# jaak-s/libfastsparse

Measured on AMD Instinct MI355X. Metric: fp64 CSR SpMV effective GB/s (% HBM3E peak), higher is better.
Workload: dtype f64

## Files before the change

### libfastsparse_amd/csrc/fs_kernels_twopass.hip

```cpp
#include <stdlib.h>

#include "fs_kernel_util.h"

namespace fs {


template <bool VALUED, int U, bool NTLD, bool NTST, int BC>
__device__ __forceinline__ void expand_share(double *__restrict__ xband, int ncol, int B, const unsigned *__restrict__ band_ptr,
                                             const uint16_t *__restrict__ lcol, const double *__restrict__ vals,
                                             const unsigned *__restrict__ gdst, const double *__restrict__ x, int xs,
                                             double *__restrict__ prod, unsigned g0, unsigned g1)
{
  const int t = threadIdx.x;
  if (g0 >= g1) return;
  int b;
  {
    int lo = 0, hi = B - 1;
    while (lo < hi) {
      const int mid = lo + ((hi - lo + 1) >> 1);
      if (band_ptr[mid] <= g0) lo = mid; else hi = mid - 1;
    }
    b = lo;
  }
  for (unsigned g = g0; g < g1; ++b) {
    const unsigned gb = band_ptr[b + 1] < g1 ? band_ptr[b + 1] : g1;
    if (gb <= g) continue;
    const int c0 = b * BC;
    const int w = (ncol - c0 < BC) ? ncol - c0 : BC;
    __syncthreads();
    {
      double r[BC / kBinBlock];
#pragma unroll
      for (int j = 0; j < BC / kBinBlock; ++j) {
        const int i = j * kBinBlock + t;
        r[j] = __builtin_nontemporal_load(x + (int64_t)(c0 + (i < w ? i : w - 1)) * xs);
      }
#pragma unroll
      for (int j = 0; j < BC / kBinBlock; ++j) {
        const int i = j * kBinBlock + t;
        xband[i] = (i < w) ? r[j] : 0.0;
      }
      if (t < 8) xband[BC + t] = 0.0;
    }
    __syncthreads();
    const int64_t e0 = (int64_t)g * kBinGroup, e1 = (int64_t)gb * kBinGroup;
    constexpr int64_t kRound = 2 * U * kBinBlock;
    int64_t o = e0 + 2 * t;
    for (; o - 2 * t + kRound <= e1; o += kRound) {
      unsigned a[U], d[U];
      v2d v[U];
#pragma unroll
      for (int k = 0; k < U; ++k) {
        const int64_t e = o + (int64_t)k * 2 * kBinBlock;
        a[k] = stream_load<NTLD>((const unsigned *)(lcol + e));
        d[k] = stream_load<NTLD>(gdst + (e >> kBinGroupLog));
        if (VALUED) v[k] = stream_load<NTLD>((const v2d *)(vals + e));
      }
      __builtin_amdgcn_sched_barrier(0);
#pragma unroll
      for (int k = 0; k < U; ++k) {
        const int64_t e = o + (int64_t)k * 2 * kBinBlock;
        v2d p = {xband[a[k] & 0xffffu], xband[a[k] >> 16]};
        if (VALUED) { p.x *= v[k].x; p.y *= v[k].y; }
        stream_store<NTST>(p, (v2d *)(prod + (int64_t)d[k] * kBinGroup + (e & (kBinGroup - 1))));
      }
    }
    for (; o < e1; o += 2 * kBinBlock) {
      const unsigned a = stream_load<NTLD>((const unsigned *)(lcol + o));
      const unsigned d = stream_load<NTLD>(gdst + (o >> kBinGroupLog));
      v2d p = {xband[a & 0xffffu], xband[a >> 16]};
      if (VALUED) {
        const v2d v = stream_load<NTLD>((const v2d *)(vals + o));
        p.x *= v.x; p.y *= v.y;
      }
      stream_store<NTST>(p, (v2d *)(prod + (int64_t)d * kBinGroup + (o & (kBinGroup - 1))));
    }
    g = gb;
  }
}

template <bool VALUED, int U, bool NTLD, bool NTST, int BC = kBinCols>
__global__ __launch_bounds__(kBinBlock) void spmv_expand_kernel(
    int ncol, int B, const unsigned *__restrict__ band_ptr, const uint16_t *__restrict__ lcol,
    const double *__restrict__ vals, const unsigned *__restrict__ gdst, const double *__restrict__ x, int xs,
    double *__restrict__ prod, unsigned gbeg, unsigned gend)
{
  __shared__ double xband[BC + 8];
  const uint64_t groups = gend - gbeg;
  const unsigned g0 = gbeg + (unsigned)(groups * blockIdx.x / gridDim.x), g1 = gbeg + (unsigned)(groups * (blockIdx.x + 1) / gridDim.x);
  expand_share<VALUED, U, NTLD, NTST, BC>(xband, ncol, B, band_ptr, lcol, vals, gdst, x, xs, prod, g0, g1);
}

template <bool NTLD, bool L8>
__device__ __forceinline__ v4u row_ids_load(const uint16_t *__restrict__ lrow, const uint8_t *__restrict__ lrow8,
                                            const uint16_t *__restrict__ gbase, int64_t e)
{
  if (!L8) return stream_load<NTLD>((const v4u *)(lrow + e));
  typedef unsigned v2u __attribute__((ext_vector_type(2)));
  const v2u d = stream_load<NTLD>((const v2u *)(lrow8 + e));
  return v4u{d.x, d.y, (unsigned)gbase[e >> kBinGroupLog], (unsigned)(e >> 3) & 1u};
}

template <bool L8>
__device__ __forceinline__ v4u row_ids(v4u raw)
{
  if (!L8) return raw;
  const unsigned dx = raw.x, dy = raw.y;
  const unsigned s0 = dx & 0xffu, s1 = s0 + ((dx >> 8) & 0xffu), s2 = s1 + ((dx >> 16) & 0xffu), s3 = s2 + (dx >> 24);
  const unsigned s4 = s3 + (dy & 0xffu), s5 = s4 + ((dy >> 8) & 0xffu), s6 = s5 + ((dy >> 16) & 0xffu), s7 = s6 + (dy >> 24);
  const unsigned below = (unsigned)__builtin_amdgcn_update_dpp(0, (int)s7, 0x111 , 0xf, 0xf, false);
  const unsigned off = raw.z + (raw.w ? below : 0u);
  return v4u{(off + s0) | ((off + s1) << 16), (off + s2) | ((off + s3) << 16), (off + s4) | ((off + s5) << 16), (off + s6) | ((off + s7) << 16)};
}

template <bool L8>
__device__ __forceinline__ unsigned line_ids_load(const uint16_t *__restrict__ lrow, const uint8_t *__restrict__ lrow8,
                                                  const uint16_t *__restrict__ gbase, int64_t e)
{
  if (!L8) return *(const unsigned *)(lrow + e);
  return (unsigned)*(const uint16_t *)(lrow8 + e) | ((unsigned)gbase[e >> kBinGroupLog] << 16);
}

template <bool L8>
__device__ __forceinline__ unsigned line_ids(unsigned raw)
{
  if (!L8) return raw;
  const unsigned d0 = raw & 0xffu, own = d0 + ((raw >> 8) & 0xffu), l = threadIdx.x & 7u;
  unsigned s = own, u;
  u = (unsigned)__builtin_amdgcn_update_dpp(0, (int)s, 0x111 , 0xf, 0xf, false); s += l >= 1 ? u : 0u;
  u = (unsigned)__builtin_amdgcn_update_dpp(0, (int)s, 0x112 , 0xf, 0xf, false); s += l >= 2 ? u : 0u;
  u = (unsigned)__builtin_amdgcn_update_dpp(0, (int)s, 0x114 , 0xf, 0xf, false); s += l >= 4 ? u : 0u;
  const unsigned off = (raw >> 16) + s - own;
  return (off + d0) | ((off + own) << 16);
}

template <bool NTLD, bool L8 = false>
__device__ __forceinline__ void reduce_panel(double *__restrict__ ytile, int panel, const unsigned *__restrict__ bin_ptr,
                                             const int *__restrict__ panel_row, const uint16_t *__restrict__ lrow,
                                             const double *__restrict__ prod, double *__restrict__ y, int ys,
                                             const uint8_t *__restrict__ lrow8 = nullptr, const uint16_t *__restrict__ gbase = nullptr)
{
  const int t = threadIdx.x;
  const int r0 = panel_row[panel], nr = panel_row[panel + 1] - r0;
  for (int i = t; i < nr; i += kBinBlock) ytile[i] = 0.0;
  __syncthreads();
  const int64_t e0 = (int64_t)bin_ptr[panel] * kBinGroup, e1 = (int64_t)bin_ptr[panel + 1] * kBinGroup;
#define FS_ADD(idx, val) __hip_atomic_fetch_add(&ytile[idx], val, __ATOMIC_RELAXED, __HIP_MEMORY_SCOPE_WORKGROUP)
#define FS_ADD2(A, P) FS_ADD((A) & 0xffffu, (P).x); FS_ADD((A) >> 16, (P).y);
  constexpr int64_t kStep = 8 * kBinBlock, kRound = 2 * kStep;
  const int wave0 = (t >> 6) * 512, lane0 = wave0 + 2 * (t & 63);
  int64_t eb = e0;
  for (; eb + kRound <= e1; eb += kRound) {
    const int64_t e = eb + lane0;
    unsigned a[2][4];
    v2d p[2][4];
#pragma unroll
    for (int k = 0; k < 2; ++k)
#pragma unroll
      for (int j = 0; j < 4; ++j) {
        const int64_t ek = e + k * kStep + 128 * j;
        a[k][j] = line_ids_load<L8>(lrow, lrow8, gbase, ek);
        p[k][j] = stream_load<NTLD>((const v2d *)(prod + ek));
      }
    __builtin_amdgcn_sched_barrier(0);
#pragma unroll
    for (int k = 0; k < 2; ++k)
#pragma unroll
      for (int j = 0; j < 4; ++j) {
        const unsigned r = line_ids<L8>(a[k][j]);
        FS_ADD2(r, p[k][j])
      }
  }
  for (; eb + wave0 < e1; eb += kStep) {
    const int64_t e = eb + lane0;
    unsigned a[4];
    v2d p[4];
#pragma unroll
    for (int j = 0; j < 4; ++j) {
      const int64_t ej = e + 128 * j, ec = ej < e1 ? ej : e1 - 2;
      a[j] = line_ids_load<L8>(lrow, lrow8, gbase, ec);
      p[j] = stream_load<NTLD>((const v2d *)(prod + ec));
    }
#pragma unroll
    for (int j = 0; j < 4; ++j) {
      const unsigned r = line_ids<L8>(a[j]);
      if (e + 128 * j < e1) { FS_ADD2(r, p[j]) }
    }
  }
#undef FS_ADD2
#undef FS_ADD
  __syncthreads();
  for (int i = t; i < nr; i += kBinBlock) y[(int64_t)(r0 + i) * ys] = ytile[i];
}

template <bool NTLD, int RM = kBinRowsMax, bool L8 = false>
__global__ __launch_bounds__(kBinBlock) void spmv_reduce_kernel(
    const unsigned *__restrict__ bin_ptr, const int *__restrict__ panel_row, const uint16_t *__restrict__ lrow,
    const double *__restrict__ prod, double *__restrict__ y, int ys, int pbase, const uint8_t *__restrict__ lrow8 = nullptr,
    const uint16_t *__restrict__ gbase = nullptr)
{
  __shared__ double ytile[RM];
  reduce_panel<NTLD, L8>(ytile, pbase + blockIdx.x, bin_ptr, panel_row, lrow, prod, y, ys, lrow8, gbase);
}

#ifndef FS_ORDERED_DEPTH
#define FS_ORDERED_DEPTH 16
#endif
template <bool NTLD, int RM, int DEPTH, bool L8 = false>
__global__ __launch_bounds__(64) void spmv_reduce_ordered_kernel(
    const unsigned *__restrict__ bin_ptr, const int *__restrict__ panel_row, const uint16_t *__restrict__ lrow,
    const double *__restrict__ prod, double *__restrict__ y, int ys, int pbase, const uint8_t *__restrict__ lrow8 = nullptr,
    const uint16_t *__restrict__ gbase = nullptr)
{
  __shared__ __attribute__((aligned(16))) double ytile[RM];
  const int t = threadIdx.x;
  const int panel = pbase + blockIdx.x;
  const int r0 = panel_row[panel], nr = panel_row[panel + 1] - r0;
  for (int i = 2 * t; i < nr; i += 128) *reinterpret_cast<v2d *>(&ytile[i]) = v2d{0.0, 0.0};
  const int64_t e0 = (int64_t)bin_ptr[panel] * kBinGroup, e1 = (int64_t)bin_ptr[panel + 1] * kBinGroup;
#define FS_ADD(idx, val) __hip_atomic_fetch_add(&ytile[idx], val, __ATOMIC_RELAXED, __HIP_MEMORY_SCOPE_WORKGROUP)
#define FS_ADD8(A, P)                                                  \
  FS_ADD(A.x & 0xffffu, P[0].x); FS_ADD(A.x >> 16, P[0].y);            \
  FS_ADD(A.y & 0xffffu, P[1].x); FS_ADD(A.y >> 16, P[1].y);            \
  FS_ADD(A.z & 0xffffu, P[2].x); FS_ADD(A.z >> 16, P[2].y);            \
  FS_ADD(A.w & 0xffffu, P[3].x); FS_ADD(A.w >> 16, P[3].y);
  constexpr int64_t kStep = 8 * 64;
  v4u a[DEPTH];
  v2d p[DEPTH][4];
  auto fetch = [&](int k, int64_t e) {
    const int64_t ec = (e + 8 <= e1) ? e : (e1 - e0 >= 8 ? e1 - 8 : e0);
    a[k] = row_ids_load<NTLD, L8>(lrow, lrow8, gbase, ec);
#pragma unroll
    for (int j = 0; j < 4; ++j) p[k][j] = stream_load<NTLD>((const v2d *)(prod + ec + 2 * j));
  };
  if (e1 > e0) {
    int64_t e = e0 + 8 * t;
#pragma unroll
    for (int k = 0; k < DEPTH; ++k) fetch(k, e + (int64_t)k * kStep);
    for (; e - 8 * t < e1; e += (int64_t)DEPTH * kStep) {
#pragma unroll
      for (int k = 0; k < DEPTH; ++k) {
        const int64_t ek = e + (int64_t)k * kStep;
        const v4u ak = row_ids<L8>(a[k]);
        v2d pk[4] = {p[k][0], p[k][1], p[k][2], p[k][3]};
        fetch(k, ek + (int64_t)DEPTH * kStep);
        if (ek + 8 <= e1) { FS_ADD8(ak, pk) }
      }
    }
  }
#undef FS_ADD8
#undef FS_ADD
  __syncthreads();
  for (int i = t; i < nr; i += 64) y[(int64_t)(r0 + i) * ys] = ytile[i];
}

template <bool VALUED, int BC, int NACC, bool ORDERED>
__global__ __launch_bounds__(kBinBlock) void spmv_longrows_kernel(
    int ncol, int B, int nlong, const int64_t *__restrict__ band_ptr, const unsigned *__restrict__ seg_ptr,
    const uint16_t *__restrict__ lcol, const uint16_t *__restrict__ lrow, const double *__restrict__ vals,
    const double *__restrict__ x, int xs, double *__restrict__ ylong, double *__restrict__ ypart)
{
  __shared__ double xband[BC + 8];
  __shared__ double acc[NACC];
  const int t = threadIdx.x, lane = t & 63, wave = t >> 6;
  for (int i = t; i < nlong; i += kBinBlock) acc[i] = 0.0;
  const int64_t pairs = band_ptr[B] >> 1;
  const int64_t e_beg = 2 * (pairs * blockIdx.x / gridDim.x), e_end = 2 * (pairs * (blockIdx.x + 1) / gridDim.x);
  if (e_beg < e_end) {
    int b;
    {
      int lo = 0, hi = B - 1;
      while (lo < hi) {
        const int mid = lo + ((hi - lo + 1) >> 1);
        if (band_ptr[mid] <= e_beg) lo = mid; else hi = mid - 1;
      }
      b = lo;
    }
    double rn[BC / kBinBlock];
    int have = -1;
    auto request = [&](int bb) {
      const int cb = bb * BC;
      const int wb = (ncol - cb < BC) ? ncol - cb : BC;
#pragma unroll
      for (int j = 0; j < BC / kBinBlock; ++j) {
        const int i = j * kBinBlock + t;
        rn[j] = __builtin_nontemporal_load(x + (int64_t)(cb + (i < wb ? i : wb - 1)) * xs);
      }
      have = bb;
    };
    auto wave_step = [&](int64_t o, bool live, int64_t oc) {
      const unsigned a = *reinterpret_cast<const unsigned *>(lcol + oc);
      const unsigned rr = *reinterpret_cast<const unsigned *>(lrow + oc);
      v2d p = {xband[a & 0xffffu], xband[a >> 16]};
      if (VALUED) { const v2d v = *reinterpret_cast<const v2d *>(vals + oc); p.x *= v.x; p.y *= v.y; }
      unsigned key = 0xffffffffu;
      double sum = 0.0;
      if (live) {
        const unsigned r0 = rr & 0xffffu, r1 = rr >> 16;
        if (r0 == r1) { key = r0; sum = p.x + p.y; }
        else { __hip_atomic_fetch_add(&acc[r0], p.x, __ATOMIC_RELAXED, __HIP_MEMORY_SCOPE_WORKGROUP); key = r1; sum = p.y; }
      }
#pragma unroll
      for (int d = 1; d < 64; d <<= 1) {
        const unsigned ku = __shfl_up(key, d);
        const double su = __shfl_up(sum, d);
        if (lane >= d && ku == key) sum += su;
      }
      const unsigned kn = __shfl_down(key, 1);
      if (live && (lane == 63 || kn != key))
        __hip_atomic_fetch_add(&acc[key], sum, __ATOMIC_RELAXED, __HIP_MEMORY_SCOPE_WORKGROUP);
      (void)o;
    };
    for (int64_t e = e_beg; e < e_end; ++b) {
      const int64_t eb = band_ptr[b + 1] < e_end ? band_ptr[b + 1] : e_end;
      if (eb <= e) continue;
      const int c0 = b * BC;
      const int w = (ncol - c0 < BC) ? ncol - c0 : BC;
      if (have != b) request(b);
      __syncthreads();
#pragma unroll
      for (int j = 0; j < BC / kBinBlock; ++j) {
        const int i = j * kBinBlock + t;
        xband[i] = (i < w) ? rn[j] : 0.0;
      }
      if (t < 8) xband[BC + t] = 0.0;
      __syncthreads();
      if (b + 1 < B && eb < e_end) request(b + 1);
      if (ORDERED) {
        const int64_t s0 = band_ptr[b] + seg_ptr[b * (kLongOwners + 1) + wave], s1 = band_ptr[b] + seg_ptr[b * (kLongOwners + 1) + wave + 1];
        const int64_t lo = s0 > e ? s0 : e, hi = s1 < eb ? s1 : eb;
        for (int64_t o0 = lo; o0 < hi; o0 += 128) {
          const int64_t o = o0 + 2 * lane;
          const bool live = o < hi;
          wave_step(o, live, live ? o : lo);
        }
      } else {
        for (int64_t o0 = e; o0 < eb; o0 += 2 * kBinBlock) {
          const int64_t o = o0 + 2 * t;
          const bool live = o < eb;
          wave_step(o, live, live ? o : e);
        }
      }
      e = eb;
    }
  }
  __syncthreads();
  if (ORDERED) {
    double *__restrict__ mine = ypart + (int64_t)blockIdx.x * nlong;
    for (int i = t; i < nlong; i += kBinBlock) mine[i] = acc[i];
  } else {
    for (int i = t; i < nlong; i += kBinBlock) {
      const double v = acc[i];
      if (v != 0.0) unsafeAtomicAdd(ylong + i, v);
    }
  }
}

__global__ __launch_bounds__(kBlock) void longrows_combine_kernel(int nlong, int nwg, const double *__restrict__ ypart, double *__restrict__ ylong)
{
  const int i = blockIdx.x * kBlock + threadIdx.x;
  if (i >= nlong) return;
  double acc = 0.0;
  for (int w = 0; w < nwg; ++w) acc += ypart[(int64_t)w * nlong + i];
  ylong[i] = acc;
}

__global__ __launch_bounds__(kBlock) void longrows_scatter_kernel(int nlong, const int *__restrict__ row, const double *__restrict__ ylong,
                                                                 double *__restrict__ y, int ys, int row0, int row1)
{
  const int i = blockIdx.x * kBlock + threadIdx.x;
  if (i >= nlong) return;
  const int r = row[i];
  if (r >= row0 && r < row1) y[(int64_t)r * ys] = 0.0 + ylong[i];
}

static int launch_longrows(const DeviceCsr &A, const LongRows &L, const double *x, int xs, hipStream_t s)
{
  const bool ordered = reproducible_now();
  if (!ordered || L.n == 0 || L.nwg == 0)
    if (int rc = launch_zero(L.ylong, sizeof(double) * (size_t)L.nlong, s)) return rc;
  if (L.n == 0 || L.nwg == 0) return FS_OK;
#define FS_LONG(V, BC, NA, ORD)                                                                                              \
  hipLaunchKernelGGL((spmv_longrows_kernel<V, BC, NA, ORD>), dim3(L.nwg), dim3(kBinBlock), 0, s, A.ncol, L.B, L.nlong, L.band_ptr, \
                     L.seg_ptr, L.lcol, L.lrow, L.vals, x, xs, L.ylong, L.ypart)
#define FS_LONG2(V, BC, NA) do { if (ordered) FS_LONG(V, BC, NA, true); else FS_LONG(V, BC, NA, false); } while (0)
  if (L.bcols == kLongBandB) { if (A.has_vals()) FS_LONG2(true, kLongBandB, kLongRowsB); else FS_LONG2(false, kLongBandB, kLongRowsB); }
  else                       { if (A.has_vals()) FS_LONG2(true, kLongBandA, kLongRowsA); else FS_LONG2(false, kLongBandA, kLongRowsA); }
#undef FS_LONG2
#undef FS_LONG
  FS_HIP(hipGetLastError());
  if (ordered) {
    hipLaunchKernelGGL(longrows_combine_kernel, dim3((unsigned)((L.nlong + kBlock - 1) / kBlock)), dim3(kBlock), 0, s, L.nlong, L.nwg, L.ypart,
                       L.ylong);
    FS_HIP(hipGetLastError());
  }
  return FS_OK;
}


template <bool VALUED, int K, int U>
__global__ __launch_bounds__(kBinBlock) void spmm_expand_kernel(
    int ncol, int B, const unsigned *__restrict__ band_ptr, const uint16_t *__restrict__ lcol,
    const double *__restrict__ vals, const unsigned *__restrict__ gdst, const double *__restrict__ X, int xs,
    double *__restrict__ prod)
{
  constexpr int BC = kBinCols / K;
  constexpr int GE = kBinGroup / K;
  constexpr int LP = K / 2;
  constexpr int EPS = kBinBlock / LP;
  __shared__ __attribute__((aligned(16))) double xband[kBinCols + 8];
  const int t = threadIdx.x;
  const int le = t / LP, h = t % LP;
  const uint64_t groups = band_ptr[B];
  const unsigned g0 = (unsigned)(groups * blockIdx.x / gridDim.x), g1 = (unsigned)(groups * (blockIdx.x + 1) / gridDim.x);
  if (g0 >= g1) return;
  int b;
  {
    int lo = 0, hi = B - 1;
    while (lo < hi) {
      const int mid = lo + ((hi - lo + 1) >> 1);
      if (band_ptr[mid] <= g0) lo = mid; else hi = mid - 1;
    }
    b = lo;
  }
  for (unsigned g = g0; g < g1; ++b) {
    const unsigned gb = band_ptr[b + 1] < g1 ? band_ptr[b + 1] : g1;
    if (gb <= g) continue;
    const int c0 = b * BC;
    const int w = (ncol - c0 < BC) ? ncol - c0 : BC;
    __syncthreads();
    {
      double r[kBinCols / kBinBlock];
#pragma unroll
      for (int j = 0; j < kBinCols / kBinBlock; ++j) {
        const int f = j * kBinBlock + t, i = f / K, q = f % K;
        r[j] = __builtin_nontemporal_load(X + (int64_t)(c0 + (i < w ? i : w - 1)) * xs + q);
      }
#pragma unroll
      for (int j = 0; j < kBinCols / kBinBlock; ++j) {
        const int f = j * kBinBlock + t;
        xband[f] = (f / K < w) ? r[j] : 0.0;
      }
      if (t < 8) xband[kBinCols + t] = 0.0;
    }
    __syncthreads();
    const int64_t e0 = (int64_t)g * GE, e1 = (int64_t)gb * GE;
    constexpr int64_t kRound = (int64_t)U * EPS;
    int64_t o = e0 + le;
    for (; o - le + kRound <= e1; o += kRound) {
      unsigned a[U], d[U];
      double v[U];
#pragma unroll
      for (int k = 0; k < U; ++k) {
        const int64_t e = o + (int64_t)k * EPS;
        a[k] = lcol[e];
        d[k] = gdst[e / GE];
        if (VALUED) v[k] = vals[e];
      }
      __builtin_amdgcn_sched_barrier(0);
#pragma unroll
      for (int k = 0; k < U; ++k) {
        const int64_t e = o + (int64_t)k * EPS;
        v2d p = *reinterpret_cast<const v2d *>(&xband[a[k] * K + 2 * h]);
        if (VALUED) { p.x *= v[k]; p.y *= v[k]; }
        __builtin_nontemporal_store(p, (v2d *)(prod + ((int64_t)d[k] * GE + (e % GE)) * K + 2 * h));
      }
    }
    for (; o < e1; o += EPS) {
      const unsigned a = lcol[o];
      const unsigned d = gdst[o / GE];
      v2d p = *reinterpret_cast<const v2d *>(&xband[a * K + 2 * h]);
      if (VALUED) { const double v = vals[o]; p.x *= v; p.y *= v; }
      __builtin_nontemporal_store(p, (v2d *)(prod + ((int64_t)d * GE + (o % GE)) * K + 2 * h));
    }
    g = gb;
  }
}

template <int K>
__global__ __launch_bounds__(kBinBlock) void spmm_reduce_kernel(
    const unsigned *__restrict__ bin_ptr_all, const int *__restrict__ panel_row_all, const uint16_t *__restrict__ lrow,
    const double *__restrict__ prod, double *__restrict__ Y, int ys, int pbase)
{
  const unsigned *__restrict__ bin_ptr = bin_ptr_all + pbase;
  const int *__restrict__ panel_row = panel_row_all + pbase;
  constexpr int GE = kBinGroup / K;
  constexpr int EPL = 8 / K;
  __shared__ double ytile[kBinRowsMax];
  const int t = threadIdx.x;
  const int r0 = panel_row[blockIdx.x], nr = panel_row[blockIdx.x + 1] - r0;
  for (int i = t; i < nr * K; i += kBinBlock) ytile[i] = 0.0;
  __syncthreads();
  const int64_t e0 = (int64_t)bin_ptr[blockIdx.x] * GE, e1 = (int64_t)bin_ptr[blockIdx.x + 1] * GE;
  typedef uint16_t rows_t __attribute__((ext_vector_type(EPL)));
#define FS_ADD(idx, val) __hip_atomic_fetch_add(&ytile[idx], val, __ATOMIC_RELAXED, __HIP_MEMORY_SCOPE_WORKGROUP)
  auto add8 = [&](const rows_t a, const v2d (&p)[4]) {
#pragma unroll
    for (int q = 0; q < EPL; ++q) {
      const int base = (int)a[q] * K;
#pragma unroll
      for (int j = 0; j < K; j += 2) {
        FS_ADD(base + j, p[(q * K + j) / 2].x);
        FS_ADD(base + j + 1, p[(q * K + j) / 2].y);
      }
    }
  };
  constexpr int64_t kStep = (int64_t)EPL * kBinBlock;
  constexpr int64_t kRound = 2 * kStep;
  int64_t e = e0 + (int64_t)EPL * t;
  for (; e - EPL * t + kRound <= e1; e += kRound) {
    rows_t a[2];
    v2d p[2][4];
#pragma unroll
    for (int k = 0; k < 2; ++k) {
      const int64_t ek = e + k * kStep;
      a[k] = *reinterpret_cast<const rows_t *>(lrow + ek);
#pragma unroll
      for (int j = 0; j < 4; ++j) p[k][j] = *reinterpret_cast<const v2d *>(prod + ek * K + 2 * j);
    }
    __builtin_amdgcn_sched_barrier(0);
    add8(a[0], p[0]);
    add8(a[1], p[1]);
  }
  for (; e < e1; e += kStep) {
    const rows_t a = *reinterpret_cast<const rows_t *>(lrow + e);
    v2d p[4];
#pragma unroll
    for (int j = 0; j < 4; ++j) p[j] = *reinterpret_cast<const v2d *>(prod + e * K + 2 * j);
    add8(a, p);
  }
#undef FS_ADD
  __syncthreads();
  for (int i = t; i < nr * K; i += kBinBlock) Y[(int64_t)(r0 + i / K) * ys + (i % K)] = ytile[i];
}

template <int K, int DEPTH>
__global__ __launch_bounds__(64) void spmm_reduce_ordered_kernel(
    const unsigned *__restrict__ bin_ptr_all, const int *__restrict__ panel_row_all, const uint16_t *__restrict__ lrow,
    const double *__restrict__ prod, double *__restrict__ Y, int ys, int pbase)
{
  const unsigned *__restrict__ bin_ptr = bin_ptr_all + pbase;
  const int *__restrict__ panel_row = panel_row_all + pbase;
  constexpr int GE = kBinGroup / K;
  constexpr int EPL = 8 / K;
  __shared__ double ytile[kBinRowsMax];
  const int t = threadIdx.x;
  const int r0 = panel_row[blockIdx.x], nr = panel_row[blockIdx.x + 1] - r0;
  for (int i = t; i < nr * K; i += 64) ytile[i] = 0.0;
  const int64_t e0 = (int64_t)bin_ptr[blockIdx.x] * GE, e1 = (int64_t)bin_ptr[blockIdx.x + 1] * GE;
  typedef uint16_t rows_t __attribute__((ext_vector_type(EPL)));
#define FS_ADD(idx, val) __hip_atomic_fetch_add(&ytile[idx], val, __ATOMIC_RELAXED, __HIP_MEMORY_SCOPE_WORKGROUP)
  auto add8 = [&](const rows_t a, const v2d (&p)[4]) {
#pragma unroll
    for (int q = 0; q < EPL; ++q) {
      const int base = (int)a[q] * K;
#pragma unroll
      for (int j = 0; j < K; j += 2) {
        FS_ADD(base + j, p[(q * K + j) / 2].x);
        FS_ADD(base + j + 1, p[(q * K + j) / 2].y);
      }
    }
  };
  constexpr int64_t kStep = (int64_t)EPL * 64;
  rows_t a[DEPTH];
  v2d p[DEPTH][4];
  auto fetch = [&](int k, int64_t e) {
    const int64_t ec = (e + EPL <= e1) ? e : (e1 - e0 >= EPL ? e1 - EPL : e0);
    a[k] = *reinterpret_cast<const rows_t *>(lrow + ec);
#pragma unroll
    for (int j = 0; j < 4; ++j) p[k][j] = *reinterpret_cast<const v2d *>(prod + ec * K + 2 * j);
  };
  if (e1 > e0) {
    int64_t e = e0 + (int64_t)EPL * t;
#pragma unroll
    for (int k = 0; k < DEPTH; ++k) fetch(k, e + (int64_t)k * kStep);
    for (; e - EPL * t < e1; e += (int64_t)DEPTH * kStep) {
#pragma unroll
      for (int k = 0; k < DEPTH; ++k) {
        const int64_t ek = e + (int64_t)k * kStep;
        const rows_t ak = a[k];
        const v2d pk[4] = {p[k][0], p[k][1], p[k][2], p[k][3]};
        fetch(k, ek + (int64_t)DEPTH * kStep);
        if (ek + EPL <= e1) add8(ak, pk);
      }
    }
  }
#undef FS_ADD
  __syncthreads();
  for (int i = t; i < nr * K; i += 64) Y[(int64_t)(r0 + i / K) * ys + (i % K)] = ytile[i];
}

template <int K>
__global__ __launch_bounds__(kBlock) void tiled_combine_k_kernel(int nrow, const int *__restrict__ vfirst,
                                                                const double *__restrict__ yv, double *__restrict__ Y, int ys,
                                                                int row0 = 0)
{
  const int64_t i = (int64_t)row0 * K + (int64_t)blockIdx.x * kBlock + threadIdx.x;
  const int64_t r = i / K;
  const int j = (int)(i % K);
  if (r >= nrow) return;
  const int a = vfirst[r], b = vfirst[r + 1];
  double acc = yv[(int64_t)a * K + j];
  for (int v = a + 1; v < b; ++v) acc += yv[(int64_t)v * K + j];
  Y[r * ys + j] = acc;
}

__global__ void rows8_decode_kernel(int64_t groups, const uint8_t *__restrict__ lrow8, const uint16_t *__restrict__ gbase,
                                    uint16_t *__restrict__ lrow)
{
  const int64_t g = (int64_t)blockIdx.x * blockDim.x + threadIdx.x;
  if (g >= groups) return;
  const v4u d = *(const v4u *)(lrow8 + g * kBinGroup);
  unsigned r = gbase[g];
  unsigned out[kBinGroup / 2];
#pragma unroll
  for (int j = 0; j < kBinGroup; j += 2) {
    const unsigned w = j < 4 ? d.x : j < 8 ? d.y : j < 12 ? d.z : d.w;
    const unsigned a = r + ((w >> (8 * (j & 3))) & 0xffu), b = a + ((w >> (8 * ((j + 1) & 3))) & 0xffu);
    out[j / 2] = a | (b << 16);
    r = b;
  }
#pragma unroll
  for (int j = 0; j < kBinGroup / 8; ++j)
    *(v4u *)(lrow + g * kBinGroup + 8 * j) = v4u{out[4 * j], out[4 * j + 1], out[4 * j + 2], out[4 * j + 3]};
}

static void ensure_two_byte_ids(BinnedCsr &N, hipStream_t s)
{
  if (N.lrow || !N.lrow8 || N.lrow_tried) return;
  hipStreamCaptureStatus cap = hipStreamCaptureStatusNone;
  if (hipStreamIsCapturing(s, &cap) != hipSuccess) { (void)hipGetLastError(); return; }
  if (cap != hipStreamCaptureStatusNone) return;
  N.lrow_tried = true;
  uint16_t *p = nullptr;
  if (hipMalloc(&p, sizeof(uint16_t) * (size_t)N.n) != hipSuccess) { (void)hipGetLastError(); return; }
  const int64_t groups = N.n >> kBinGroupLog;
  if (groups > 0) hipLaunchKernelGGL(rows8_decode_kernel, dim3((unsigned)((groups + 255) / 256)), dim3(256), 0, s, groups, N.lrow8, N.gbase, p);
  if (hipGetLastError() != hipSuccess || hipStreamSynchronize(s) != hipSuccess) { (void)hipGetLastError(); (void)hipFree(p); return; }
  N.lrow = p;
}

static void launch_reduce(const BinnedCsr &N, double *out, int os, int p0, int p1, int flags, hipStream_t s)
{
#define FS_REDUCE(NT, RM, L8)                                                                                               \
  hipLaunchKernelGGL((spmv_reduce_kernel<NT, RM, L8>), dim3(p1 - p0), dim3(kBinBlock), 0, s, N.bin_ptr, N.panel_row, N.lrow, \
                     N.prod, out, os, p0, N.lrow8, N.gbase)
#define FS_REDUCE2(RM, L8) do { if (flags & 256) FS_REDUCE(false, RM, L8); else FS_REDUCE(true, RM, L8); } while (0)
  if (N.bcols == kBinColsBig) FS_REDUCE2(kBinRowsBig, false);
  else if (N.lrow8)           FS_REDUCE2(kBinRowsMax, true);
  else                        FS_REDUCE2(kBinRowsMax, false);
#undef FS_REDUCE2
#undef FS_REDUCE
}

int launch_spmv_binned(const DeviceCsr &A, double *y, const double *x, hipStream_t s, int xs, int ys, int p0, int p1, int row0,
                       int row1)
{
  const BinnedCsr &N = *A.binned;
  double *out = N.split ? N.yv : y;
  const int os = N.split ? 1 : ys;
  const bool part = p1 >= 0;
  if (!part) { p0 = 0; p1 = N.P; row0 = 0; row1 = A.nrow; }
  const int nwg1 = (options().bin_wgs > 0 && options().bin_wgs < N.nwg1) ? options().bin_wgs : N.nwg1;
  if (nwg1 > 0 && p0 == 0) {
    const int flags = options().bin_flags;
#define FS_EXPAND4(V, U)                                                                                          \
  do {                                                                                                            \
    if (flags & 16) { if (flags & 8) FS_EXPAND(V, U, true, false);  else FS_EXPAND(V, U, true, true); }           \
    else            { if (flags & 8) FS_EXPAND(V, U, false, false); else FS_EXPAND(V, U, false, true); }          \
  } while (0)
#define FS_EXPAND(V, U, NL, NS)                                                                                    \
  hipLaunchKernelGGL((spmv_expand_kernel<V, U, NL, NS>), dim3(nwg1), dim3(kBinBlock), 0, s, A.ncol, N.B, N.band_ptr, \
                     N.lcol, N.vals, N.gdst, x, xs, N.prod, 0u, (unsigned)(N.n >> kBinGroupLog))
    if (N.bcols == kBinColsBig) {
      if (A.has_vals())
        hipLaunchKernelGGL((spmv_expand_kernel<true, 4, false, true, kBinColsBig>), dim3(nwg1), dim3(kBinBlock), 0, s, A.ncol, N.B,
                           N.band_ptr, N.lcol, N.vals, N.gdst, x, xs, N.prod, 0u, (unsigned)(N.n >> kBinGroupLog));
      else
        hipLaunchKernelGGL((spmv_expand_kernel<false, 4, false, true, kBinColsBig>), dim3(nwg1), dim3(kBinBlock), 0, s, A.ncol, N.B,
                           N.band_ptr, N.lcol, N.vals, N.gdst, x, xs, N.prod, 0u, (unsigned)(N.n >> kBinGroupLog));
    } else
    if (A.has_vals()) { if ((flags & 3) == 1) FS_EXPAND4(true, 8); else if ((flags & 3) == 2) FS_EXPAND4(true, 2); else FS_EXPAND4(true, 4); }
    else        { if ((flags & 3) == 1) FS_EXPAND4(false, 8); else if ((flags & 3) == 2) FS_EXPAND4(false, 2); else FS_EXPAND4(false, 4); }
#undef FS_EXPAND4
#undef FS_EXPAND
    FS_HIP(hipGetLastError());
  }
  if (N.lr && p0 == 0)
    if (int rc = launch_longrows(A, *N.lr, x, xs, s)) return rc;
  if (p1 > p0) {
    const bool ordered = reproducible_now() || (options().bin_flags & 32);
    if (ordered && N.lrow8 && !N.lrow) ensure_two_byte_ids(*A.binned, s);
    if (N.bcols == kBinColsBig && ordered)
      hipLaunchKernelGGL((spmv_reduce_ordered_kernel<false, kBinRowsBig, FS_ORDERED_DEPTH>), dim3(p1 - p0), dim3(64), 0, s, N.bin_ptr,
                         N.panel_row, N.lrow, N.prod, out, os, p0);
    else if (ordered && N.lrow8 && !N.lrow)
      hipLaunchKernelGGL((spmv_reduce_ordered_kernel<false, kBinRowsMax, FS_ORDERED_DEPTH, true>), dim3(p1 - p0), dim3(64), 0, s, N.bin_ptr,
                         N.panel_row, N.lrow, N.prod, out, os, p0, N.lrow8, N.gbase);
    else if (ordered)
      hipLaunchKernelGGL((spmv_reduce_ordered_kernel<false, kBinRowsMax, FS_ORDERED_DEPTH>), dim3(p1 - p0), dim3(64), 0, s, N.bin_ptr,
                         N.panel_row, N.lrow, N.prod, out, os, p0);
    else
      launch_reduce(N, out, os, p0, p1, options().bin_flags, s);
    FS_HIP(hipGetLastError());
  }
  if (N.split && row1 > row0) {
    if (int rc = launch_tiled_combine(row1, N.vfirst, N.yv, y, ys, row0, s)) return rc;
  }
  if (N.lr && row1 > row0) {
    hipLaunchKernelGGL(longrows_scatter_kernel, dim3((unsigned)((N.lr->nlong + kBlock - 1) / kBlock)), dim3(kBlock), 0, s, N.lr->nlong,
                       N.lr->row, N.lr->ylong, y, ys, row0, row1);
    FS_HIP(hipGetLastError());
  }
  return FS_OK;
}

int launch_expand_groups(const DeviceCsr &A, const double *x, unsigned g0, unsigned g1, int wgs, hipStream_t s)
{
  const BinnedCsr &N = *A.binned;
  if (g1 <= g0 || wgs <= 0) return FS_OK;
#define FS_XH(V, BC)                                                                                                    \
  hipLaunchKernelGGL((spmv_expand_kernel<V, 4, false, true, BC>), dim3(wgs), dim3(kBinBlock), 0, s, A.ncol, N.B, N.band_ptr, \
                     N.lcol, N.vals, N.gdst, x, 1, N.prod, g0, g1)
  if (N.bcols == kBinColsBig) { if (A.has_vals()) FS_XH(true, kBinColsBig); else FS_XH(false, kBinColsBig); }
  else                        { if (A.has_vals()) FS_XH(true, kBinCols); else FS_XH(false, kBinCols); }
#undef FS_XH
  FS_HIP(hipGetLastError());
  return FS_OK;
}

int launch_reduce_panels(const DeviceCsr &A, double *y, int p0, int p1, hipStream_t s)
{
  const BinnedCsr &N = *A.binned;
  if (p1 <= p0) return FS_OK;
  launch_reduce(N, y, 1, p0, p1, 0, s);
  FS_HIP(hipGetLastError());
  return FS_OK;
}

int launch_spmm_binned(const DeviceCsr &A, const BinnedCsr &N, double *Y, const double *X, hipStream_t s, int xs, int ys, int p0,
                       int p1, int row0, int row1)
{
  const int K = N.kw;
  double *out = N.split ? N.yv : Y;
  const int os = N.split ? K : ys;
  if (p1 < 0) { p0 = 0; p1 = N.P; row0 = 0; row1 = A.nrow; }
  const int nwg1 = (p0 != 0) ? 0 : ((options().bin_wgs > 0 && options().bin_wgs < N.nwg1) ? options().bin_wgs : N.nwg1);
#define FS_XP(V, KK)                                                                                                  \
  hipLaunchKernelGGL((spmm_expand_kernel<V, KK, 4>), dim3(nwg1), dim3(kBinBlock), 0, s, A.ncol, N.B, N.band_ptr, N.lcol, \
                     N.vals, N.gdst, X, xs, N.prod)
  if (nwg1 > 0) {
    if (K == 2) { if (A.has_vals()) FS_XP(true, 2); else FS_XP(false, 2); }
    else        { if (A.has_vals()) FS_XP(true, 4); else FS_XP(false, 4); }
    FS_HIP(hipGetLastError());
  }
#undef FS_XP
  if (p1 > p0) {
    const bool ordered = reproducible_now() || (options().bin_flags & 32);
    if (K == 2 && ordered)
      hipLaunchKernelGGL((spmm_reduce_ordered_kernel<2, FS_ORDERED_DEPTH>), dim3(p1 - p0), dim3(64), 0, s, N.bin_ptr, N.panel_row, N.lrow, N.prod, out, os, p0);
    else if (ordered)
      hipLaunchKernelGGL((spmm_reduce_ordered_kernel<4, FS_ORDERED_DEPTH>), dim3(p1 - p0), dim3(64), 0, s, N.bin_ptr, N.panel_row, N.lrow, N.prod, out, os, p0);
    else if (K == 2)
      hipLaunchKernelGGL(spmm_reduce_kernel<2>, dim3(p1 - p0), dim3(kBinBlock), 0, s, N.bin_ptr, N.panel_row, N.lrow, N.prod, out, os, p0);
    else
      hipLaunchKernelGGL(spmm_reduce_kernel<4>, dim3(p1 - p0), dim3(kBinBlock), 0, s, N.bin_ptr, N.panel_row, N.lrow, N.prod, out, os, p0);
    FS_HIP(hipGetLastError());
  }
  if (N.split && row1 > row0) {
    const unsigned grid = (unsigned)(((int64_t)(row1 - row0) * K + kBlock - 1) / kBlock);
    if (K == 2)
      hipLaunchKernelGGL(tiled_combine_k_kernel<2>, dim3(grid), dim3(kBlock), 0, s, row1, N.vfirst, N.yv, Y, ys, row0);
    else
      hipLaunchKernelGGL(tiled_combine_k_kernel<4>, dim3(grid), dim3(kBlock), 0, s, row1, N.vfirst, N.yv, Y, ys, row0);
    FS_HIP(hipGetLastError());
  }
  return FS_OK;
}

}
```

Before: 2595.

## Split expand load cache hints per stream and restructure SpMM reduce loads

After: 2590. About the same (-0.2%).

```diff
diff --git a/libfastsparse_amd/csrc/fs_kernels_twopass.hip b/libfastsparse_amd/csrc/fs_kernels_twopass.hip
--- a/libfastsparse_amd/csrc/fs_kernels_twopass.hip
+++ b/libfastsparse_amd/csrc/fs_kernels_twopass.hip
@@ -5,7 +5,10 @@
 namespace fs {
 
 
-template <bool VALUED, int U, bool NTLD, bool NTST, int BC>
+constexpr bool kExpandValsNT = false, kExpandLcolNT = false;
+constexpr bool kSpmmValsNT = false, kSpmmLcolNT = false;
+
+template <bool VALUED, int U, bool NTV, bool NTC, bool NTST, int BC>
 __device__ __forceinline__ void expand_share(double *__restrict__ xband, int ncol, int B, const unsigned *__restrict__ band_ptr,
                                              const uint16_t *__restrict__ lcol, const double *__restrict__ vals,
                                              const unsigned *__restrict__ gdst, const double *__restrict__ x, int xs,
@@ -52,9 +55,9 @@
 #pragma unroll
       for (int k = 0; k < U; ++k) {
         const int64_t e = o + (int64_t)k * 2 * kBinBlock;
-        a[k] = stream_load<NTLD>((const unsigned *)(lcol + e));
-        d[k] = stream_load<NTLD>(gdst + (e >> kBinGroupLog));
-        if (VALUED) v[k] = stream_load<NTLD>((const v2d *)(vals + e));
+        a[k] = stream_load<NTC>((const unsigned *)(lcol + e));
+        d[k] = gdst[e >> kBinGroupLog];
+        if (VALUED) v[k] = stream_load<NTV>((const v2d *)(vals + e));
       }
       __builtin_amdgcn_sched_barrier(0);
 #pragma unroll
@@ -66,11 +69,11 @@
       }
     }
     for (; o < e1; o += 2 * kBinBlock) {
-      const unsigned a = stream_load<NTLD>((const unsigned *)(lcol + o));
-      const unsigned d = stream_load<NTLD>(gdst + (o >> kBinGroupLog));
+      const unsigned a = stream_load<NTC>((const unsigned *)(lcol + o));
+      const unsigned d = gdst[o >> kBinGroupLog];
       v2d p = {xband[a & 0xffffu], xband[a >> 16]};
       if (VALUED) {
-        const v2d v = stream_load<NTLD>((const v2d *)(vals + o));
+        const v2d v = stream_load<NTV>((const v2d *)(vals + o));
         p.x *= v.x; p.y *= v.y;
       }
       stream_store<NTST>(p, (v2d *)(prod + (int64_t)d * kBinGroup + (o & (kBinGroup - 1))));
@@ -79,7 +82,7 @@
   }
 }
 
-template <bool VALUED, int U, bool NTLD, bool NTST, int BC = kBinCols>
+template <bool VALUED, int U, bool NTV, bool NTC, bool NTST, int BC = kBinCols>
 __global__ __launch_bounds__(kBinBlock) void spmv_expand_kernel(
     int ncol, int B, const unsigned *__restrict__ band_ptr, const uint16_t *__restrict__ lcol,
     const double *__restrict__ vals, const unsigned *__restrict__ gdst, const double *__restrict__ x, int xs,
@@ -88,7 +91,7 @@
   __shared__ double xband[BC + 8];
   const uint64_t groups = gend - gbeg;
   const unsigned g0 = gbeg + (unsigned)(groups * blockIdx.x / gridDim.x), g1 = gbeg + (unsigned)(groups * (blockIdx.x + 1) / gridDim.x);
-  expand_share<VALUED, U, NTLD, NTST, BC>(xband, ncol, B, band_ptr, lcol, vals, gdst, x, xs, prod, g0, g1);
+  expand_share<VALUED, U, NTV, NTC, NTST, BC>(xband, ncol, B, band_ptr, lcol, vals, gdst, x, xs, prod, g0, g1);
 }
 
 template <bool NTLD, bool L8>
@@ -398,7 +401,7 @@
 }
 
 
-template <bool VALUED, int K, int U>
+template <bool VALUED, int K, int U, bool NTV, bool NTC>
 __global__ __launch_bounds__(kBinBlock) void spmm_expand_kernel(
     int ncol, int B, const unsigned *__restrict__ band_ptr, const uint16_t *__restrict__ lcol,
     const double *__restrict__ vals, const unsigned *__restrict__ gdst, const double *__restrict__ X, int xs,
@@ -453,9 +456,9 @@
 #pragma unroll
       for (int k = 0; k < U; ++k) {
         const int64_t e = o + (int64_t)k * EPS;
-        a[k] = lcol[e];
+        a[k] = stream_load<NTC>(lcol + e);
         d[k] = gdst[e / GE];
-        if (VALUED) v[k] = vals[e];
+        if (VALUED) v[k] = stream_load<NTV>(vals + e);
       }
       __builtin_amdgcn_sched_barrier(0);
 #pragma unroll
@@ -467,17 +470,17 @@
       }
     }
     for (; o < e1; o += EPS) {
-      const unsigned a = lcol[o];
+      const unsigned a = stream_load<NTC>(lcol + o);
       const unsigned d = gdst[o / GE];
       v2d p = *reinterpret_cast<const v2d *>(&xband[a * K + 2 * h]);
-      if (VALUED) { const double v = vals[o]; p.x *= v; p.y *= v; }
+      if (VALUED) { const double v = stream_load<NTV>(vals + o); p.x *= v; p.y *= v; }
       __builtin_nontemporal_store(p, (v2d *)(prod + ((int64_t)d * GE + (o % GE)) * K + 2 * h));
     }
     g = gb;
   }
 }
 
-template <int K>
+template <int K, bool NTLD>
 __global__ __launch_bounds__(kBinBlock) void spmm_reduce_kernel(
     const unsigned *__restrict__ bin_ptr_all, const int *__restrict__ panel_row_all, const uint16_t *__restrict__ lrow,
     const double *__restrict__ prod, double *__restrict__ Y, int ys, int pbase)
@@ -485,50 +488,52 @@
   const unsigned *__restrict__ bin_ptr = bin_ptr_all + pbase;
   const int *__restrict__ panel_row = panel_row_all + pbase;
   constexpr int GE = kBinGroup / K;
-  constexpr int EPL = 8 / K;
+  constexpr int KLOG = K == 2 ? 1 : 2;
+  static_assert(K == 2 || K == 4, "a lane owns one pair of an entry's K products");
   __shared__ double ytile[kBinRowsMax];
   const int t = threadIdx.x;
   const int r0 = panel_row[blockIdx.x], nr = panel_row[blockIdx.x + 1] - r0;
   for (int i = t; i < nr * K; i += kBinBlock) ytile[i] = 0.0;
   __syncthreads();
-  const int64_t e0 = (int64_t)bin_ptr[blockIdx.x] * GE, e1 = (int64_t)bin_ptr[blockIdx.x + 1] * GE;
-  typedef uint16_t rows_t __attribute__((ext_vector_type(EPL)));
+  const int64_t d0 = (int64_t)bin_ptr[blockIdx.x] * GE * K, d1 = (int64_t)bin_ptr[blockIdx.x + 1] * GE * K;
 #define FS_ADD(idx, val) __hip_atomic_fetch_add(&ytile[idx], val, __ATOMIC_RELAXED, __HIP_MEMORY_SCOPE_WORKGROUP)
-  auto add8 = [&](const rows_t a, const v2d (&p)[4]) {
-#pragma unroll
-    for (int q = 0; q < EPL; ++q) {
-      const int base = (int)a[q] * K;
-#pragma unroll
-      for (int j = 0; j < K; j += 2) {
-        FS_ADD(base + j, p[(q * K + j) / 2].x);
-        FS_ADD(base + j + 1, p[(q * K + j) / 2].y);
-      }
-    }
-  };
-  constexpr int64_t kStep = (int64_t)EPL * kBinBlock;
-  constexpr int64_t kRound = 2 * kStep;
-  int64_t e = e0 + (int64_t)EPL * t;
-  for (; e - EPL * t + kRound <= e1; e += kRound) {
-    rows_t a[2];
+#define FS_ADD2(R, D, P) { const int base = (int)(R) * K + (int)((D) & (K - 1)); FS_ADD(base, (P).x); FS_ADD(base + 1, (P).y); }
+  constexpr int64_t kStep = 8 * kBinBlock, kRound = 2 * kStep;
+  const int wave0 = (t >> 6) * 512, lane0 = wave0 + 2 * (t & 63);
+  int64_t db = d0;
+  for (; db + kRound <= d1; db += kRound) {
+    const int64_t d = db + lane0;
+    unsigned a[2][4];
     v2d p[2][4];
 #pragma unroll
-    for (int k = 0; k < 2; ++k) {
-      const int64_t ek = e + k * kStep;
-      a[k] = *reinterpret_cast<const rows_t *>(lrow + ek);
-#pragma unroll
-      for (int j = 0; j < 4; ++j) p[k][j] = *reinterpret_cast<const v2d *>(prod + ek * K + 2 * j);
-    }
+    for (int k = 0; k < 2; ++k)
+#pragma unroll
+      for (int j = 0; j < 4; ++j) {
+        const int64_t dk = d + k * kStep + 128 * j;
+        a[k][j] = lrow[dk >> KLOG];
+        p[k][j] = stream_load<NTLD>((const v2d *)(prod + dk));
+      }
     __builtin_amdgcn_sched_barrier(0);
-    add8(a[0], p[0]);
-    add8(a[1], p[1]);
-  }
-  for (; e < e1; e += kStep) {
-    const rows_t a = *reinterpret_cast<const rows_t *>(lrow + e);
+#pragma unroll
+    for (int k = 0; k < 2; ++k)
+#pragma unroll
+      for (int j = 0; j < 4; ++j) FS_ADD2(a[k][j], d + 128 * j, p[k][j])
+  }
+  for (; db + wave0 < d1; db += kStep) {
+    const int64_t d = db + lane0;
+    unsigned a[4];
     v2d p[4];
 #pragma unroll
-    for (int j = 0; j < 4; ++j) p[j] = *reinterpret_cast<const v2d *>(prod + e * K + 2 * j);
-    add8(a, p);
-  }
+    for (int j = 0; j < 4; ++j) {
+      const int64_t dj = d + 128 * j, dc = dj < d1 ? dj : d1 - 2;
+      a[j] = lrow[dc >> KLOG];
+      p[j] = stream_load<NTLD>((const v2d *)(prod + dc));
+    }
+#pragma unroll
+    for (int j = 0; j < 4; ++j)
+      if (d + 128 * j < d1) FS_ADD2(a[j], d + 128 * j, p[j])
+  }
+#undef FS_ADD2
 #undef FS_ADD
   __syncthreads();
   for (int i = t; i < nr * K; i += kBinBlock) Y[(int64_t)(r0 + i / K) * ys + (i % K)] = ytile[i];
@@ -664,25 +669,33 @@
   const int nwg1 = (options().bin_wgs > 0 && options().bin_wgs < N.nwg1) ? options().bin_wgs : N.nwg1;
   if (nwg1 > 0 && p0 == 0) {
     const int flags = options().bin_flags;
-#define FS_EXPAND4(V, U)                                                                                          \
+    const bool ntv = kExpandValsNT != !!(flags & 512), ntc = kExpandLcolNT != !!(flags & 1024);
+#define FS_EXPAND(V, U, NV, NC, NS)                                                                                        \
+  hipLaunchKernelGGL((spmv_expand_kernel<V, U, NV, NC, NS>), dim3(nwg1), dim3(kBinBlock), 0, s, A.ncol, N.B, N.band_ptr, \
+                     N.lcol, N.vals, N.gdst, x, xs, N.prod, 0u, (unsigned)(N.n >> kBinGroupLog))
+#define FS_EXPAND_ST(V, U) do { if (flags & 8) FS_EXPAND(V, U, kExpandValsNT, kExpandLcolNT, false); else FS_EXPAND(V, U, kExpandValsNT, kExpandLcolNT, true); } while (0)
+#define FS_EXPAND_LD(V)                                                                                            \
   do {                                                                                                            \
-    if (flags & 16) { if (flags & 8) FS_EXPAND(V, U, true, false);  else FS_EXPAND(V, U, true, true); }           \
-    else            { if (flags & 8) FS_EXPAND(V, U, false, false); else FS_EXPAND(V, U, false, true); }          \
+    if (ntv && V) { if (ntc) FS_EXPAND(V, 4, V, true, true);  else FS_EXPAND(V, 4, V, false, true); }               \
+    else          { if (ntc) FS_EXPAND(V, 4, false, true, true); else FS_EXPAND(V, 4, false, false, true); }      \
   } while (0)
-#define FS_EXPAND(V, U, NL, NS)                                                                                    \
-  hipLaunchKernelGGL((spmv_expand_kernel<V, U, NL, NS>), dim3(nwg1), dim3(kBinBlock), 0, s, A.ncol, N.B, N.band_ptr, \
-                     N.lcol, N.vals, N.gdst, x, xs, N.prod, 0u, (unsigned)(N.n >> kBinGroupLog))
+#define FS_EXPAND_ALL(V)                                                                                           \
+  do {                                                                                                            \
+    if ((flags & 3) == 1) FS_EXPAND_ST(V, 8); else if ((flags & 3) == 2) FS_EXPAND_ST(V, 2);                       \
+    else if (flags & 8) FS_EXPAND_ST(V, 4); else FS_EXPAND_LD(V);                                                  \
+  } while (0)
     if (N.bcols == kBinColsBig) {
       if (A.has_vals())
-        hipLaunchKernelGGL((spmv_expand_kernel<true, 4, false, true, kBinColsBig>), dim3(nwg1), dim3(kBinBlock), 0, s, A.ncol, N.B,
-                           N.band_ptr, N.lcol, N.vals, N.gdst, x, xs, N.prod, 0u, (unsigned)(N.n >> kBinGroupLog));
+        hipLaunchKernelGGL((spmv_expand_kernel<true, 4, kExpandValsNT, kExpandLcolNT, true, kBinColsBig>), dim3(nwg1), dim3(kBinBlock), 0, s,
+                           A.ncol, N.B, N.band_ptr, N.lcol, N.vals, N.gdst, x, xs, N.prod, 0u, (unsigned)(N.n >> kBinGroupLog));
       else
-        hipLaunchKernelGGL((spmv_expand_kernel<false, 4, false, true, kBinColsBig>), dim3(nwg1), dim3(kBinBlock), 0, s, A.ncol, N.B,
-                           N.band_ptr, N.lcol, N.vals, N.gdst, x, xs, N.prod, 0u, (unsigned)(N.n >> kBinGroupLog));
+        hipLaunchKernelGGL((spmv_expand_kernel<false, 4, false, kExpandLcolNT, true, kBinColsBig>), dim3(nwg1), dim3(kBinBlock), 0, s,
+                           A.ncol, N.B, N.band_ptr, N.lcol, N.vals, N.gdst, x, xs, N.prod, 0u, (unsigned)(N.n >> kBinGroupLog));
     } else
-    if (A.has_vals()) { if ((flags & 3) == 1) FS_EXPAND4(true, 8); else if ((flags & 3) == 2) FS_EXPAND4(true, 2); else FS_EXPAND4(true, 4); }
-    else        { if ((flags & 3) == 1) FS_EXPAND4(false, 8); else if ((flags & 3) == 2) FS_EXPAND4(false, 2); else FS_EXPAND4(false, 4); }
-#undef FS_EXPAND4
+    if (A.has_vals()) FS_EXPAND_ALL(true); else FS_EXPAND_ALL(false);
+#undef FS_EXPAND_ALL
+#undef FS_EXPAND_LD
+#undef FS_EXPAND_ST
 #undef FS_EXPAND
     FS_HIP(hipGetLastError());
   }
@@ -720,8 +733,8 @@
   const BinnedCsr &N = *A.binned;
   if (g1 <= g0 || wgs <= 0) return FS_OK;
 #define FS_XH(V, BC)                                                                                                    \
-  hipLaunchKernelGGL((spmv_expand_kernel<V, 4, false, true, BC>), dim3(wgs), dim3(kBinBlock), 0, s, A.ncol, N.B, N.band_ptr, \
-                     N.lcol, N.vals, N.gdst, x, 1, N.prod, g0, g1)
+  hipLaunchKernelGGL((spmv_expand_kernel<V, 4, V && kExpandValsNT, kExpandLcolNT, true, BC>), dim3(wgs), dim3(kBinBlock), 0, s, A.ncol, \
+                     N.B, N.band_ptr, N.lcol, N.vals, N.gdst, x, 1, N.prod, g0, g1)
   if (N.bcols == kBinColsBig) { if (A.has_vals()) FS_XH(true, kBinColsBig); else FS_XH(false, kBinColsBig); }
   else                        { if (A.has_vals()) FS_XH(true, kBinCols); else FS_XH(false, kBinCols); }
 #undef FS_XH
@@ -746,25 +759,34 @@
   const int os = N.split ? K : ys;
   if (p1 < 0) { p0 = 0; p1 = N.P; row0 = 0; row1 = A.nrow; }
   const int nwg1 = (p0 != 0) ? 0 : ((options().bin_wgs > 0 && options().bin_wgs < N.nwg1) ? options().bin_wgs : N.nwg1);
-#define FS_XP(V, KK)                                                                                                  \
-  hipLaunchKernelGGL((spmm_expand_kernel<V, KK, 4>), dim3(nwg1), dim3(kBinBlock), 0, s, A.ncol, N.B, N.band_ptr, N.lcol, \
+  const int flags = options().bin_flags;
+  const bool ntv = kSpmmValsNT != !!(flags & 512), ntc = kSpmmLcolNT != !!(flags & 1024);
+#define FS_XP(V, KK, NV, NC)                                                                                                  \
+  hipLaunchKernelGGL((spmm_expand_kernel<V, KK, 4, NV, NC>), dim3(nwg1), dim3(kBinBlock), 0, s, A.ncol, N.B, N.band_ptr, N.lcol, \
                      N.vals, N.gdst, X, xs, N.prod)
+#define FS_XP2(V, KK)                                                                               \
+  do {                                                                                              \
+    if (ntv && V) { if (ntc) FS_XP(V, KK, V, true); else FS_XP(V, KK, V, false); }                  \
+    else          { if (ntc) FS_XP(V, KK, false, true); else FS_XP(V, KK, false, false); }          \
+  } while (0)
   if (nwg1 > 0) {
-    if (K == 2) { if (A.has_vals()) FS_XP(true, 2); else FS_XP(false, 2); }
-    else        { if (A.has_vals()) FS_XP(true, 4); else FS_XP(false, 4); }
+    if (K == 2) { if (A.has_vals()) FS_XP2(true, 2); else FS_XP2(false, 2); }
+    else        { if (A.has_vals()) FS_XP2(true, 4); else FS_XP2(false, 4); }
     FS_HIP(hipGetLastError());
   }
+#undef FS_XP2
 #undef FS_XP
   if (p1 > p0) {
     const bool ordered = reproducible_now() || (options().bin_flags & 32);
+#define FS_RK(KK, NT) \
+  hipLaunchKernelGGL((spmm_reduce_kernel<KK, NT>), dim3(p1 - p0), dim3(kBinBlock), 0, s, N.bin_ptr, N.panel_row, N.lrow, N.prod, out, os, p0)
     if (K == 2 && ordered)
       hipLaunchKernelGGL((spmm_reduce_ordered_kernel<2, FS_ORDERED_DEPTH>), dim3(p1 - p0), dim3(64), 0, s, N.bin_ptr, N.panel_row, N.lrow, N.prod, out, os, p0);
     else if (ordered)
       hipLaunchKernelGGL((spmm_reduce_ordered_kernel<4, FS_ORDERED_DEPTH>), dim3(p1 - p0), dim3(64), 0, s, N.bin_ptr, N.panel_row, N.lrow, N.prod, out, os, p0);
-    else if (K == 2)
-      hipLaunchKernelGGL(spmm_reduce_kernel<2>, dim3(p1 - p0), dim3(kBinBlock), 0, s, N.bin_ptr, N.panel_row, N.lrow, N.prod, out, os, p0);
-    else
-      hipLaunchKernelGGL(spmm_reduce_kernel<4>, dim3(p1 - p0), dim3(kBinBlock), 0, s, N.bin_ptr, N.panel_row, N.lrow, N.prod, out, os, p0);
+    else if (K == 2) { if (options().bin_flags & 256) FS_RK(2, false); else FS_RK(2, true); }
+    else             { if (options().bin_flags & 256) FS_RK(4, false); else FS_RK(4, true); }
+#undef FS_RK
     FS_HIP(hipGetLastError());
   }
   if (N.split && row1 > row0) {
```
